# Shunpoco/mini-kube-scheduler

Measured on AMD Instinct MI355X. Metric: pod×node filter+score evals/sec and pods scheduled/sec at 100k nodes, 1/2/4/8 GPU, higher is better.
Workload: dtype u32; 1 GPU; C: 100000 nodes x 100000 pods (100000 per GPU, strong scaling), NU+NN, batched, every pair evaluated, node-sharded over 1 GPU; nodes=100000, pods=100000, pods_per_gpu=100000, plugins=NU+NN, parallelism=node-shard1

## Files before the change

mini-kube-scheduler_amd/csrc/ms_sweep_pp.hip:

```cpp
#include <hip/hip_ext.h>

#include <algorithm>
#include <cstdlib>

#include "ms_device.h"

namespace msgpu {

namespace {

template <typename F>
constexpr uint32_t truth3(F f) {
    uint32_t t = 0;
    for (int i = 0; i < 8; ++i)
        if (f((i >> 2) & 1, (i >> 1) & 1, i & 1)) t |= 1u << i;
    return t;
}
constexpr uint32_t kXnorAnd = truth3([](int a, int b, int c) { return c && a == b; });
constexpr uint32_t kSelect = truth3([](int a, int b, int c) { return c ? a : b; });

constexpr uint32_t kTailShare = 4;

constexpr int kPpWords = 4;
constexpr int kPpWordsSmall = 8;
constexpr int kPpMaxWaves = 16;
constexpr uint32_t kPpSmallGroups = 64u * kPpWordsSmall;

struct Word {
    uint32_t d0, d1, d2, d3;
    uint32_t sched, pres;
    uint32_t dsched, dpres;
    uint32_t hb;
};

struct Pod {
    uint32_t A;
    uint32_t s0, s1, s2, s3;
    uint32_t tol;
    uint32_t p0, p1, p2;
    uint32_t A0, A1, A2;
};

#define MS_BITOP3(a, b, c, imm) __builtin_amdgcn_bitop3_b32((a), (b), (c), (imm))

__device__ __forceinline__ uint32_t feasible(const Word &w, const Pod &q) {
    return MS_BITOP3(w.pres, w.sched, q.tol, kSelect);
}

__device__ __forceinline__ uint32_t match10(const Word &w, const Pod &q) {
    uint32_t m = MS_BITOP3(w.d0, q.s0, feasible(w, q), kXnorAnd);
    m = MS_BITOP3(w.d1, q.s1, m, kXnorAnd);
    m = MS_BITOP3(w.d2, q.s2, m, kXnorAnd);
    return MS_BITOP3(w.d3, q.s3, m, kXnorAnd);
}

__device__ __forceinline__ uint32_t last_lz(uint32_t m) {
    uint32_t s;
    asm("v_ffbh_u32 %0, %1" : "=v"(s) : "v"(m));
// ... 214 lines not shown
    uint32_t off, ns, nt;
};

__device__ __forceinline__ DigitLists digit_lists(const uint32_t *hdr, uint32_t d) {
    DigitLists L;
    L.off = hdr[d];
    L.nt = (hdr[d + 1] - L.off) / kCandTile;
    L.ns = hdr[kCandDigits + 1u + d];
    return L;
}

__device__ __forceinline__ uint32_t list_tiles(const DigitLists &L, bool tolerates) {
    return tolerates ? L.nt : L.ns;
}

struct ClassLanes {
    uint32_t beg, end;
    DigitLists L;
    u64 planes;
};

__device__ __forceinline__ ClassLanes class_lanes(const uint32_t *hdr, const uint32_t *rb, uint32_t base10,
                                                  uint32_t lane) {
    const uint32_t c = min(lane, kPpClasses);
    ClassLanes C;
    C.beg = rb[c];
    C.end = rb[c + 1];
    C.L = digit_lists(hdr, ((c >> 1) + base10) % kCandDigits);
    C.planes = __ballot(lane <= kPpClasses && C.beg < C.end &&
                        (c == kPpClasses || list_tiles(C.L, (c & 1u) != 0u) == 0u));
    return C;
}

__device__ __forceinline__ uint32_t lane_value(uint32_t v, uint32_t l) {
    return (uint32_t)__builtin_amdgcn_readlane((int)v, (int)l);
}

template <int NT>
__device__ __forceinline__ void sweep_list_pods(const uint32_t (&B)[3 * kPpWords], const uint2 *pinfo, uint32_t beg,
                                                uint32_t end, uint32_t lane, u64 *lds) {
    for (uint32_t pb = beg; pb < end; pb += 64) {
        const uint32_t nblk = min(64u, end - pb);
        const uint32_t a_l = lane < nblk ? pinfo[pb + lane].x : 0u;
        for (uint32_t j = 0; j < nblk; j += 8) {
            uint32_t r[8];
            if (nblk - j >= 8u) {
#pragma unroll
                for (int t = 0; t < 8; ++t) {
                    const uint32_t A = (uint32_t)__builtin_amdgcn_readlane((int)a_l, (int)(j + t));
                    uint32_t h = 0;
#pragma unroll
                    for (int i = 0; i < 3 * NT; ++i) h = max(h, mix32(B[i] + A));
                    r[t] = h;
                }
            } else {
#pragma unroll
                for (int t = 0; t < 8; ++t) {
                    r[t] = 0;
                    if (j + (uint32_t)t < nblk) {
                        const uint32_t A = (uint32_t)__builtin_amdgcn_readlane((int)a_l, (int)(j + t));
#pragma unroll
                        for (int i = 0; i < 3 * NT; ++i) r[t] = max(r[t], mix32(B[i] + A));
                    }
                }
            }
            const uint32_t u = reduce8(r, lane);
            const uint32_t pi = j + rev3(lane >> 3);
            if ((lane & 7u) == 0u && pi < nblk) atomicMax(&lds[pb + pi], (11ull << 32) | u);
        }
    }
}

__device__ __forceinline__ void sweep_list_tiles(uint32_t n, const uint32_t (&B)[3 * kPpWords], const uint2 *pinfo,
                                                 uint32_t beg, uint32_t end, uint32_t lane, u64 *lds) {
    switch (n) {
        case 1: sweep_list_pods<1>(B, pinfo, beg, end, lane, lds); break;
        case 2: sweep_list_pods<2>(B, pinfo, beg, end, lane, lds); break;
        case 3: sweep_list_pods<3>(B, pinfo, beg, end, lane, lds); break;
        default: sweep_list_pods<4>(B, pinfo, beg, end, lane, lds); break;
    }
}

__device__ __forceinline__ void load_list_tiles(const uint32_t *__restrict__ cand, uint32_t off, uint32_t t0,
                                                uint32_t nt, uint32_t waves, uint32_t lane,
                                                uint32_t (&B)[3 * kPpWords]) {
#pragma unroll
    for (int k = 0; k < kPpWords; ++k) {
        const uint32_t tile = t0 + ((uint32_t)k < nt ? (uint32_t)k * waves : 0u);
        const uint32_t *e = cand + kCandHeader + off + tile * kCandTile + lane;
#pragma unroll
        for (int i = 0; i < 3; ++i) B[3 * k + i] = e[i * 64];
    }
}

__device__ __forceinline__ void sweep_lists(const uint32_t *__restrict__ cand, const ClassLanes &C,
                                            const uint2 *pinfo, uint32_t wv, uint32_t waves, uint32_t lane,
                                            u64 *lds) {
    for (uint32_t s = 0; s < kPpClasses; s += 2) {
        const uint32_t b0 = lane_value(C.beg, s), b1 = lane_value(C.end, s), b2 = lane_value(C.end, s + 1u);
        if (b0 >= b2) continue;
        const DigitLists L = {lane_value(C.L.off, s), lane_value(C.L.ns, s), lane_value(C.L.nt, s)};
        const uint32_t ntile = list_tiles(L, b1 < b2);
        for (uint32_t t0 = wv; t0 < ntile; t0 += kPpWords * waves) {
            const uint32_t nt = min((uint32_t)kPpWords, (ntile - t0 + waves - 1u) / waves);
            const uint32_t ns = t0 < L.ns ? min((uint32_t)kPpWords, (L.ns - t0 + waves - 1u) / waves) : 0u;
            uint32_t B[3 * kPpWords];
            load_list_tiles(cand, L.off, t0, nt, waves, lane, B);
            if (ns != 0u && b0 < b1) sweep_list_tiles(ns, B, pinfo, b0, b1, lane, lds);
            if (b1 < b2) sweep_list_tiles(nt, B, pinfo, b1, b2, lane, lds);
        }
    }
}

template <int KW, int NW, int MODE, bool TAIL>
__device__ __forceinline__ void sweep_range(const Word (&W)[KW], const Word &Wt, uint32_t tpt, uint32_t tshare,
                                            uint32_t tidx, const uint2 *pinfo, const uint32_t *rb, bool runs,
                                            bool lists, const uint32_t *hdr, uint32_t base10, uint32_t np,
                                            uint32_t lane, u64 *lds) {
    constexpr bool RUN = MODE != kModeGen && NW > 0 && KW == kPpWords;
    const bool cut = lists || (RUN && runs);
    u64 todo = cut ? (2ull << kPpClasses) - 1ull : 1ull << kPpClasses;
    uint32_t cbeg = 0, cend = 0;
    if (lists) {
        const ClassLanes C = class_lanes(hdr, rb, base10, lane);
        cbeg = C.beg, cend = C.end, todo = C.planes;
    }
    for (; todo; todo &= todo - 1ull) {
        const uint32_t c = (uint32_t)__builtin_ctzll(todo);
        const uint32_t beg = lists ? lane_value(cbeg, c)
                             : cut ? (uint32_t)__builtin_amdgcn_readfirstlane((int)rb[c]) : 0u;
        const uint32_t end = lists ? lane_value(cend, c)
                             : cut ? (uint32_t)__builtin_amdgcn_readfirstlane((int)rb[c + 1]) : np;
        if (beg >= end) continue;
        uint32_t B[RUN ? NW * 3 : 1] = {};
        bool form = false;
        if constexpr (RUN)
            if (!lists && c < kPpClasses)
                form = run_setup<KW, NW>(W, (uint32_t)__builtin_amdgcn_readfirstlane((int)pinfo[beg].y), B);
        sweep_pods<KW, NW, MODE, TAIL>(W, Wt, tpt, tshare, tidx, pinfo, beg, end, form, B, lane, lds);
    }
}

__host__ __device__ inline uint32_t tail_pods(uint32_t ng, uint32_t waves) {
    if (ng == 0) return 0u;
    const uint32_t wlast = (ng + 63u) / 64u - 1u, tail_n = ng - wlast * 64u;
    const uint32_t tpt = tail_n <= 8u ? 8u : 0u;
    if (!tpt) return 0u;
    if (waves <= 4u) return tpt;
    const uint32_t wv_t = wlast % waves;
    const uint32_t tshare = kTailShare < waves - wv_t ? kTailShare : waves - wv_t;
    uint32_t L[4] = {0, 0, 0, 0};
    for (uint32_t w = 0; w < waves && w <= wlast; ++w) L[w & 3u] += 16u * ((wlast - w) / waves + 1u);
    auto mx = [&] {
        const uint32_t a = L[0] > L[1] ? L[0] : L[1], b = L[2] > L[3] ? L[2] : L[3];
        return a > b ? a : b;
    };
    const uint32_t m0 = mx();
    L[wv_t & 3u] -= 16u;
    const uint32_t eps = ((tpt == 8u ? 4u : tpt == 4u ? 8u : 12u) + tshare - 1u) / tshare;
    for (uint32_t i = 0; i < tshare; ++i) L[(wv_t + i) & 3u] += eps;
    return mx() < m0 ? tpt : 0u;
}

struct PpJob2 {
    const ms_pod_rec *pods;
    u64 *keys;
    uint32_t n_pods, nblk1;
};

template <int KW, bool TP>
__global__ __launch_bounds__(64 * kPpMaxWaves) void k_sweep_nunn_pp(
    const uint32_t *__restrict__ planes, uint32_t gstride, uint32_t n_groups, uint32_t node_base,
    const ms_pod_rec *__restrict__ pods1, uint32_t n_pods1, uint32_t chunk, uint32_t seed32, u64 *__restrict__ keys1,
    int atomic_keys, ms_result *__restrict__ results, uint32_t present, NodeTable tab, int commit,
    uint32_t pstride, ms_result_compact *__restrict__ resc, PpJob2 j2, int fix_ok, uint32_t xtra,
    const uint32_t *__restrict__ cand) {
    extern __shared__ u64 lds[];
    uint2 *pinfo = reinterpret_cast<uint2 *>(lds + chunk + (xtra ? 8u : 0u));
    const uint32_t lane = lane_id();
    const uint32_t wv = (uint32_t)__builtin_amdgcn_readfirstlane((int)(threadIdx.x >> 6));
    const bool second = j2.pods && blockIdx.x >= j2.nblk1;
    const ms_pod_rec *__restrict__ pods = second ? j2.pods : pods1;
    const uint32_t n_pods = second ? j2.n_pods : n_pods1;
    u64 *__restrict__ keys = second ? j2.keys : keys1;
    const uint32_t bi = second ? blockIdx.x - j2.nblk1 : blockIdx.x;
    const uint32_t pbeg = bi * chunk + min(bi, xtra) * 8u;
    const uint32_t pend = min(n_pods, pbeg + chunk + (bi < xtra ? 8u : 0u));
    const uint32_t np = pend > pbeg ? pend - pbeg : 0u;
    uint32_t *cnt = reinterpret_cast<uint32_t *>(pinfo + chunk + (xtra ? 8u : 0u));
    uint32_t *rb = cnt + 24, *sb = cnt + 48, *hdr = cnt + 72;
    const bool runs = KW == kPpWords && chunk >= kPpSortMin;
    const bool lists = runs && cand != nullptr && gridDim.y == 1u;
    if (!runs) {
        for (uint32_t i = threadIdx.x; i < np; i += blockDim.x) {
            lds[i] = 0;
            uint2 e = pod_entry(pods, pbeg + i, seed32, pstride, node_base % 10u);
            e.y |= i << 21;
            pinfo[i] = e;
        }
    } else {
        if (threadIdx.x < 24u) cnt[threadIdx.x] = 0u;
        if (lists)
            for (uint32_t i = threadIdx.x; i <= kCandClasses; i += blockDim.x) hdr[i] = cand[i];
        __syncthreads();
        for (uint32_t i = threadIdx.x; i < np; i += blockDim.x) {
            uint2 e = pod_entry(pods, pbeg + i, seed32, pstride, node_base % 10u);
            e.y |= atomicAdd(&cnt[pod_class(e.y)], 1u) << 21;
            reinterpret_cast<uint2 *>(lds)[i] = e;
        }
        __syncthreads();
        if (threadIdx.x <= kPpClasses) {
            uint32_t a = 0, b = 0, na = 0, nb = 0;
            for (uint32_t c = 0; c < kPpClasses; ++c) {
                const uint32_t n = cnt[c], full = lists ? n : n & ~7u;
                if (c == threadIdx.x) a = na, b = nb;
                na += full;
                nb += n - full;
            }
            if (threadIdx.x == kPpClasses) {
                a = na, b = nb;
                rb[kPpClasses + 1] = np;
            }
            rb[threadIdx.x] = a;
            sb[threadIdx.x] = na + b;
        }
        __syncthreads();
        for (uint32_t i = threadIdx.x; i < np; i += blockDim.x) {
            const uint2 e = reinterpret_cast<const uint2 *>(lds)[i];
            const uint32_t c = pod_class(e.y), rank = e.y >> 21;
            const uint32_t full = c < kPpClasses ? rb[c + 1] - rb[c] : 0u;
            const uint32_t pos = rank < full ? rb[c] + rank : sb[c] + (rank - full);
            pinfo[pos] = make_uint2(e.x, (e.y & 0x1FFFFFu) | (i << 21));
            lds[i] = 0;
        }
    }

    const uint32_t waves = blockDim.x >> 6;
    const uint32_t g0 = blockIdx.y * waves * 64u * KW;
    const uint32_t ng = min(n_groups - g0, waves * 64u * KW);
    const uint32_t wlast = (ng + 63u) / 64u - 1u, tail_n = ng - wlast * 64u;
    uint32_t tpt = TP ? tail_pods(ng, waves) : 0u;
    const uint32_t wv_t = wlast % waves, tshare = min(kTailShare, waves - wv_t);
    const bool owner = wv == wv_t;
    if (wv < wv_t || wv >= wv_t + tshare) tpt = 0u;
    Word W[KW], Wt;
    int nw = 0;
    bool over = false, misaligned = false;
#pragma unroll
    for (int k = 0; k < KW; ++k) {
        const uint32_t wi = k * waves + wv;
        const uint32_t gw = g0 + wi * 64u;
        const uint32_t g = gw + lane;
        const bool in = g < n_groups && !(tpt && owner && wi == wlast);
        if (gw < n_groups && !(tpt && owner && wi == wlast)) nw = k + 1;
        W[k].d0 = in ? planes[kPlaneD0 * gstride + g] : 0u;
        W[k].d1 = in ? planes[kPlaneD1 * gstride + g] : 0u;
        W[k].d2 = in ? planes[kPlaneD2 * gstride + g] : 0u;
        W[k].d3 = in ? planes[kPlaneD3 * gstride + g] : 0u;
        W[k].sched = in ? planes[kPlaneSched * gstride + g] : 0u;
        W[k].pres = in ? planes[kPlanePresent * gstride + g] : 0u;
        W[k].dsched = in ? planes[kPlaneDigitSched * gstride + g] : 0u;
        W[k].dpres = in ? planes[kPlaneDigitPres * gstride + g] : 0u;
        W[k].hb = (node_base + g * kGroupRows) * kG24;
        const uint32_t ov = in ? planes[kPlaneOver * gstride + g] : 0u;
        over = over || (ov & 1u) != 0u;
        misaligned = misaligned || (ov & 2u) != 0u;
    }
    {
        const uint32_t gi = tpt ? lane & ((64u / tpt) - 1u) : 0u;
        const uint32_t g = g0 + wlast * 64u + gi;
        const bool in = tpt && gi < tail_n;
        Wt.d0 = in ? planes[kPlaneD0 * gstride + g] : 0u;
        Wt.d1 = in ? planes[kPlaneD1 * gstride + g] : 0u;
        Wt.d2 = in ? planes[kPlaneD2 * gstride + g] : 0u;
        Wt.d3 = in ? planes[kPlaneD3 * gstride + g] : 0u;
        Wt.sched = in ? planes[kPlaneSched * gstride + g] : 0u;
        Wt.pres = in ? planes[kPlanePresent * gstride + g] : 0u;
        Wt.hb = (node_base + g * kGroupRows) * kG24;
        Wt.dsched = Wt.dpres = 0u;
        over = over || (in && (planes[kPlaneOver * gstride + g] & 1u) != 0u);
    }
    const bool gen = __ballot(over) != 0;
    const int mode = gen ? kModeGen : (fix_ok && __ballot(misaligned) == 0) ? kModeFix : kModeFast;
    __syncthreads();
    if (np && (nw || tpt)) {
        switch (nw * 6 + mode * 2 + (tpt ? 1 : 0)) {
#define MS_PP_CASE1(N, M, T)                                                                                     \
    case 6 * N + 2 * M + T:                                                                                      \
        if constexpr (N <= KW && (N > 0 || T))                                                                   \
            sweep_range<KW, (N <= KW ? N : KW), M, T>(W, Wt, tpt, tshare, wv - wv_t, pinfo, rb, runs, lists, hdr,   \
                                                      node_base % 10u, np, lane, lds);                          \
        break;
#define MS_PP_CASE(N)        \
    MS_PP_CASE1(N, 0, false) \
    MS_PP_CASE1(N, 0, true)  \
    MS_PP_CASE1(N, 1, false) \
    MS_PP_CASE1(N, 1, true)  \
    MS_PP_CASE1(N, 2, false) \
    MS_PP_CASE1(N, 2, true)
            MS_PP_CASE(0)
            MS_PP_CASE(1)
            MS_PP_CASE(2)
            MS_PP_CASE(3)
            MS_PP_CASE(4)
            MS_PP_CASE(5)
            MS_PP_CASE(6)
            MS_PP_CASE(7)
            MS_PP_CASE(8)
#undef MS_PP_CASE
#undef MS_PP_CASE1
            default:
                break;
        }
    }
    if constexpr (KW == kPpWords)
        if (np && lists)
            sweep_lists(cand, class_lanes(hdr, rb, node_base % 10u, lane), pinfo, wv, waves, lane, lds);
    __syncthreads();
    for (uint32_t i = threadIdx.x; i < np; i += blockDim.x) {
        const u64 v = lds[i];
        const uint2 pe = pinfo[i];
        const uint32_t po = pbeg + (pe.y >> 21);
        u64 key = present ? kKeyListed : 0ull;
        if (v) {
            const uint32_t h = (uint32_t)v;
            key = make_key((uint32_t)(v >> 32) - 1u, h, tb_unhash(pe.x, h));
        }
        if (keys) {
            if (!atomic_keys) keys[po] = key;
            else if (key) atomicMax(&keys[po], key);
        }
        if (results || resc) {
            const ms_result r = decode_key(key, (int8_t)(pe.y >> 8), nullptr, 0, present);
            if (results) {
                results[po] = r;
            } else {
                ms_result_compact rc;
                rc.node = r.node;
                rc.score = (uint16_t)r.score;
                rc.code = (uint8_t)r.code;
                rc.plugin_mask = (uint8_t)r.plugin_mask;
                resc[po] = rc;
            }
            if (commit && r.code == MS_CODE_SUCCESS) {
                if (resc) {
                    const ms_pod_rec z = {};
                    add_pod(tab, (uint32_t)r.node - tab.base, z, +1);
                } else {
                    add_pod(tab, (uint32_t)r.node - tab.base, pods[po], +1);
                }
            }
        }
    }
}

__host__ __device__ inline uint32_t cdiv(uint32_t a, uint32_t b) { return (a + b - 1) / b; }

__device__ __forceinline__ void build_group(const NodeTable &t, uint32_t g) {
    uint32_t d[4] = {0, 0, 0, 0}, sched = 0, pres = 0, isdig = 0, misal = 0;
    for (uint32_t s = 0; s < kGroupRows; ++s) {
        const uint32_t r = g * kGroupRows + s;
        if (r >= t.cap) break;
        const uint32_t f = t.flags[r], dg = t.digit[r];
        const uint32_t v = dg <= 9u ? dg : 15u;
#pragma unroll
        for (int b = 0; b < 4; ++b) d[b] |= ((v >> b) & 1u) << s;
        if (!(f & kNodeAbsent)) {
            pres |= 1u << s;
            if (!(f & kNodeUnschedulable)) sched |= 1u << s;
            if (v <= 9u) {
                isdig |= 1u << s;
                if (v != (t.base + r) % 10u) misal = 2u;
            }
        }
    }
    uint32_t over = misal;
#pragma unroll
    for (int v = 0; v < 10; ++v) {
        const uint32_t m = pres & ((v & 1) ? d[0] : ~d[0]) & ((v & 2) ? d[1] : ~d[1]) & ((v & 4) ? d[2] : ~d[2]) &
                           ((v & 8) ? d[3] : ~d[3]);
        over |= __popc(m) > 3 ? 1u : 0u;
    }
    const uint32_t st = t.gcap;
    t.planes[kPlaneDigitPres * st + g] = pres & isdig;
    t.planes[kPlaneDigitSched * st + g] = sched & isdig;
    t.planes[kPlaneOver * st + g] = over;
// ... 73 lines not shown
            total += wsum[w];
        }
        uint32_t pos = done + before + incl - k;
        while (m) {
            const uint32_t slot = (uint32_t)__builtin_ctz(m);
            m &= m - 1u;
            const uint32_t e = (t.base + g * kGroupRows + slot) * kG24;
            if (pos == 0u) first = e;
            if (pos < len) ent[pos] = e;
            ++pos;
        }
        done += total;
        __syncthreads();
    }
    for (uint32_t i = len + tid; i < padded; i += kCandThreads) ent[i] = first;
}

}

hipError_t launch_build_planes(const NodeTable &t, uint32_t *cand, const NodeDelta *d_deltas, uint32_t n,
                               hipStream_t s) {
    if (!t.planes) return hipSuccess;
    if (!d_deltas) n = t.gcap;
    if (n == 0) return hipSuccess;
    hipLaunchKernelGGL(k_build_planes, dim3(cdiv(n, 256)), dim3(256), 0, s, t, d_deltas, n);
    hipError_t e = hipGetLastError();
    if (e != hipSuccess || !cand) return e;
    hipLaunchKernelGGL(k_build_cand, dim3(kCandClasses), dim3(kCandThreads), 0, s, t, cand);
    return hipGetLastError();
}

constexpr uint32_t kPpMaxChunk = 2048;

namespace {
hipError_t sweep_pp_impl(const NodeTable &t, const uint32_t *cand, uint32_t n_rows, const ms_pod_rec *pods, uint32_t n_pods,
                         uint32_t seed32, unsigned long long *keys, ms_result *results, uint32_t present, int num_cus,
                         hipStream_t s, int commit, hipEvent_t done, uint32_t pstride, ms_result_compact *resc,
                         const ms_pod_rec *pods2 = nullptr, uint32_t n_pods2 = 0, unsigned long long *keys2 = nullptr) {
    if (n_pods == 0 && n_pods2 == 0) return done ? hipEventRecord(done, s) : hipSuccess;
    const uint32_t n_all = n_pods + (pods2 ? n_pods2 : 0u);
    if (!t.planes) return hipErrorInvalidValue;
    const uint32_t n_groups = cdiv(n_rows, kGroupRows);
    const char *wenv = getenv("MINISCHED_PP_WORDS");
    const uint32_t cus_ = (uint32_t)(num_cus > 0 ? num_cus : 256);
    bool small = n_groups <= kPpSmallGroups && n_all >= 1024u * cus_ && !getenv("MINISCHED_PP_WAVES");
    if (wenv) small = n_groups <= kPpSmallGroups && atoi(wenv) == 8;
    const uint32_t KW = small ? (uint32_t)kPpWordsSmall : (uint32_t)kPpWords;
    const uint32_t waves_needed = std::max(1u, cdiv(n_groups, 64u * KW));
    uint32_t W = 1;
    if (waves_needed == 2) W = 2;
    else if (waves_needed > 1)
        while (W < std::max(4u, waves_needed) && W < (uint32_t)kPpMaxWaves) W *= 2;
    if (const char *w = getenv("MINISCHED_PP_WAVES")) W = (uint32_t)std::min(16, std::max(1, atoi(w)));
    if (!keys) W = std::max(W, std::min<uint32_t>(kPpMaxWaves, waves_needed));
    const uint32_t gy = std::max(1u, cdiv(n_groups, W * 64u * KW));
    const uint32_t cus = (uint32_t)(num_cus > 0 ? num_cus : 256);
    auto chunk_for = [&](uint32_t per_cu) {
        const uint32_t resident = std::max(1u, per_cu * cus / gy);
        return cdiv(cdiv(n_all, resident), 8) * 8;
    };
    uint32_t chunk = chunk_for(std::max(1u, 32u / W));
    if (32u / W > 1u && chunk_for(std::max(1u, 16u / W)) <= 1024u) chunk = chunk_for(std::max(1u, 16u / W));
    chunk = std::min(std::max(chunk, 8u), kPpMaxChunk);
    uint32_t nblk1 = cdiv(n_pods, chunk), xtra = 0;
    if ((!pods2 || n_pods2 == n_pods) && gy == 1 && W <= 4u) {
        const uint32_t slots = (16u / W) * cus / (pods2 ? 2u : 1u);
        const uint32_t cb = (n_pods / slots) / 8u * 8u;
        if (cb >= 8u && cb + 8u <= kPpMaxChunk && n_pods > cb * slots) {
            const uint32_t nx = cdiv(n_pods - cb * slots, 8u);
            if (nx <= slots) {
                chunk = cb;
                xtra = nx;
                nblk1 = slots;
            }
        }
    }
    const dim3 grid(nblk1 + (pods2 ? (xtra ? nblk1 : cdiv(n_pods2, chunk)) : 0u), gy);
    constexpr int fix_ok = 1;
    const PpJob2 j2 = {pods2, reinterpret_cast<u64 *>(keys2), n_pods2, nblk1};
    if (pods2 && (gy > 1 || results || resc || !keys || !keys2)) return hipErrorInvalidValue;
    if (gy > 1) {
        if (!keys || resc) return hipErrorInvalidValue;
        hipError_t e = hipMemsetAsync(keys, 0, sizeof(unsigned long long) * n_pods, s);
        if (e != hipSuccess) return e;
        hipLaunchKernelGGL((k_sweep_nunn_pp<kPpWords, false>), grid, dim3(64 * W),
                           chunk * (sizeof(u64) + sizeof(uint2)) + kPpSortWords * sizeof(uint32_t), s, t.planes,
                           t.gcap, n_groups, t.base, pods, n_pods, chunk, seed32, keys, 1, (ms_result *)nullptr, present,
                           t, 0, (uint32_t)sizeof(ms_pod_rec), (ms_result_compact *)nullptr, PpJob2{}, fix_ok, 0u,
                           (const uint32_t *)nullptr);
        e = hipGetLastError();
        if (e == hipSuccess && results) e = launch_decode(pods, n_pods, keys, nullptr, present, results, s);
        if (e == hipSuccess && results && commit) e = launch_apply_binds(t, pods, n_pods, results, s);
        if (e == hipSuccess && done) e = hipEventRecord(done, s);
        return e;
    }
    const uint32_t lds = (chunk + (xtra ? 8u : 0u)) * (sizeof(u64) + sizeof(uint2)) + kPpSortWords * sizeof(uint32_t);
    unsigned long long *kk = (results || resc) ? nullptr : keys;
    const int cm = (results || resc) ? commit : 0;
    const bool tp = KW == (uint32_t)kPpWords && tail_pods(n_groups, W) != 0u;
#define MS_PP_LAUNCH(KWV, TPV)                                                                                     \
    hipExtLaunchKernelGGL((k_sweep_nunn_pp<KWV, TPV>), grid, dim3(64 * W), lds, s, nullptr, done, 0, t.planes, t.gcap, \
                          n_groups, t.base, pods, n_pods, chunk, seed32, kk, 0, results, present, t, cm, pstride, resc, j2, \
                          fix_ok, xtra, cand)
    if (KW == (uint32_t)kPpWordsSmall) {
        MS_PP_LAUNCH(kPpWordsSmall, false);
    } else {
        if (tp) MS_PP_LAUNCH(kPpWords, true);
        else MS_PP_LAUNCH(kPpWords, false);
    }
#undef MS_PP_LAUNCH
    return hipGetLastError();
}
}

hipError_t launch_sweep_pp(const NodeTable &t, const uint32_t *cand, uint32_t n_rows, const ms_pod_rec *pods, uint32_t n_pods,
                           uint32_t seed32, unsigned long long *keys, ms_result *results, uint32_t present,
                           int num_cus, hipStream_t s, int commit, hipEvent_t done) {
    return sweep_pp_impl(t, cand, n_rows, pods, n_pods, seed32, keys, results, present, num_cus, s, commit, done,
                         (uint32_t)sizeof(ms_pod_rec), nullptr);
}

hipError_t launch_sweep_pp2(const NodeTable &t, const uint32_t *cand, uint32_t n_rows, const ms_pod_rec *pods1, uint32_t n1,
                            unsigned long long *keys1, const ms_pod_rec *pods2, uint32_t n2, unsigned long long *keys2,
                            uint32_t seed32, uint32_t present, int num_cus, hipStream_t s, hipEvent_t done) {
    if (n_rows > kPpMaxFusedRows) return hipErrorInvalidValue;
    return sweep_pp_impl(t, cand, n_rows, pods1, n1, seed32, keys1, nullptr, present, num_cus, s, 0, done,
                         (uint32_t)sizeof(ms_pod_rec), nullptr, pods2, n2, keys2);
}

hipError_t launch_sweep_pp_compact(const NodeTable &t, const uint32_t *cand, uint32_t n_rows, const ms_pod_compact *pods, uint32_t n_pods,
                                   uint32_t seed32, ms_result_compact *results, uint32_t present, int num_cus,
                                   hipStream_t s) {
    static_assert(sizeof(ms_pod_compact) == 8 && sizeof(ms_result_compact) == 8, "compact records");
    if (n_rows > kPpMaxFusedRows || !results) return hipErrorInvalidValue;
    return sweep_pp_impl(t, cand, n_rows, reinterpret_cast<const ms_pod_rec *>(pods), n_pods, seed32, nullptr, nullptr,
                         present, num_cus, s, 1, nullptr, (uint32_t)sizeof(ms_pod_compact), results);
}

}
```

Before: 57270 billion pod×node evals/s.

## Deal list tiles and pod ranges across wave groups in sweep_lists

Waves are now split into up to four groups. Each group takes a share of the pod blocks per digit, rotated between digits so the load stays balanced, and each wave holds up to G×4 candidate tiles in registers instead of 4. The intent is more register reuse of the loaded tiles across pods and fewer redundant tile loads per pod. The cost is higher register pressure from larger B arrays, which may hurt occupancy, plus a runtime-looped tail path. The change also adds optional timeline instrumentation that is compiled out by default.

After: 59650 billion pod×node evals/s, median of 6. +4.1%, better.

```diff
diff --git a/mini-kube-scheduler_amd/csrc/ms_pp_deal.h b/mini-kube-scheduler_amd/csrc/ms_pp_deal.h
--- /dev/null
+++ b/mini-kube-scheduler_amd/csrc/ms_pp_deal.h
@@ -0,0 +1,105 @@
+#pragma once
+
+#include <cstdint>
+
+#if !defined(__HIPCC__) && !defined(__host__)
+#define __host__
+#define __device__
+#define MS_PP_DEAL_OWN_ATTRS
+#endif
+
+namespace msgpu {
+
+constexpr uint32_t kDealTiles = 4;
+
+struct WaveDeal {
+    uint32_t groups;
+    uint32_t gshift;
+    uint32_t group;
+    uint32_t index;
+    uint32_t wpg;
+    uint32_t inv;
+};
+
+__host__ __device__ inline uint32_t deal_groups(uint32_t waves, uint32_t want) {
+    if (waves % 4u) return 1u;
+    uint32_t g = want >= 4u ? 4u : want >= 2u ? 2u : 1u;
+    while (g > 1u && (waves / 4u) % g) g >>= 1;
+    return g;
+}
+
+__host__ __device__ inline WaveDeal wave_deal(uint32_t wv, uint32_t waves, uint32_t want) {
+    WaveDeal D;
+    D.groups = deal_groups(waves, want);
+    D.gshift = D.groups >> 1;
+    D.group = (wv >> 2) & (D.groups - 1u);
+    D.index = (wv & 3u) + 4u * ((wv >> 2) >> D.gshift);
+    D.wpg = waves >> D.gshift;
+    D.inv = 0xFFFFFFFFu / D.wpg + 1u;
+    return D;
+}
+
+__host__ __device__ inline uint32_t deal_div(const WaveDeal &D, uint32_t n) {
+    return D.wpg == 1u ? n : (uint32_t)(((unsigned long long)n * D.inv) >> 32);
+}
+
+__host__ __device__ inline uint32_t deal_hold(const WaveDeal &D) { return kDealTiles << D.gshift; }
+__host__ __device__ inline uint32_t deal_pass_tiles(const WaveDeal &D) { return deal_hold(D) * D.wpg; }
+
+struct DigitDeal {
+    uint32_t off, nt, ns;
+};
+
+__host__ __device__ inline DigitDeal deal_digit(const WaveDeal &D, uint32_t ntile, uint32_t ns_all) {
+    DigitDeal X;
+    X.off = D.index;
+    const uint32_t qt = deal_div(D, ntile), rt = ntile - qt * D.wpg;
+    const uint32_t qs = deal_div(D, ns_all), rs = ns_all - qs * D.wpg;
+    X.nt = qt + (X.off < rt ? 1u : 0u);
+    X.ns = qs + (X.off < rs ? 1u : 0u);
+    return X;
+}
+
+struct TileDeal {
+    uint32_t first, nt, ns;
+};
+
+__host__ __device__ inline TileDeal deal_tiles(const WaveDeal &D, const DigitDeal &X, uint32_t pass) {
+    const uint32_t hold = deal_hold(D), done = pass * hold;
+    TileDeal T;
+    T.first = done * D.wpg + X.off;
+    T.nt = X.nt > done ? X.nt - done : 0u;
+    if (T.nt > hold) T.nt = hold;
+    T.ns = X.ns > done ? X.ns - done : 0u;
+    if (T.ns > T.nt) T.ns = T.nt;
+    return T;
+}
+
+struct PodDeal {
+    uint32_t beg, end;
+};
+
+__host__ __device__ inline PodDeal deal_pods(const WaveDeal &D, uint32_t prot, uint32_t beg, uint32_t end) {
+    const uint32_t nb = end > beg ? (end - beg + 7u) >> 3 : 0u;
+    const uint32_t base = nb >> D.gshift, extra = nb & (D.groups - 1u);
+    const uint32_t gi = (D.group - prot) & (D.groups - 1u);
+    const uint32_t start = gi * base + (gi < extra ? gi : extra), cnt = base + (gi < extra ? 1u : 0u);
+    PodDeal P;
+    P.beg = beg + 8u * start;
+    P.end = beg + 8u * (start + cnt);
+    if (P.end > end) P.end = end;
+    if (cnt == 0u || P.beg > P.end) P.beg = P.end;
+    return P;
+}
+
+__host__ __device__ inline uint32_t deal_prot_next(const WaveDeal &D, uint32_t prot, uint32_t n) {
+    return (prot + ((n + 7u) >> 3)) & (D.groups - 1u);
+}
+
+}
+
+#ifdef MS_PP_DEAL_OWN_ATTRS
+#undef __host__
+#undef __device__
+#undef MS_PP_DEAL_OWN_ATTRS
+#endif
diff --git a/mini-kube-scheduler_amd/csrc/ms_sweep_pp.hip b/mini-kube-scheduler_amd/csrc/ms_sweep_pp.hip
--- a/mini-kube-scheduler_amd/csrc/ms_sweep_pp.hip
+++ b/mini-kube-scheduler_amd/csrc/ms_sweep_pp.hip
@@ -4,10 +4,36 @@
 #include <cstdlib>
 
 #include "ms_device.h"
+#include "ms_pp_deal.h"
+
+#ifdef MS_PP_TIMELINE
+#include <cstdio>
+#include <vector>
+#endif
 
 namespace msgpu {
 
 namespace {
+
+#ifdef MS_PP_TIMELINE
+constexpr uint32_t kTlEntry = 0, kTlSorted = 1, kTlPlanes = 2, kTlBarrier = 3, kTlPlaneSweep = 4;
+constexpr uint32_t kTlDigit = 5;
+constexpr uint32_t kTlDone = 35, kTlFinalBarrier = 36, kTlExit = 37, kTlHwId = 38, kTlSlots = 40;
+__device__ unsigned long long *g_pp_tl;
+__device__ __forceinline__ void pp_stamp(uint32_t slot, bool hwid = false) {
+    unsigned long long *tl = g_pp_tl;
+    if (!tl) return;
+    const uint32_t waves = blockDim.x >> 6, wg = blockIdx.x * gridDim.y + blockIdx.y;
+    const unsigned long long t =
+        hwid ? (unsigned long long)__builtin_amdgcn_s_getreg((31 << 11) | 4) : __builtin_amdgcn_s_memrealtime();
+    if ((threadIdx.x & 63u) == 0u) tl[((size_t)wg * waves + (threadIdx.x >> 6)) * kTlSlots + slot] = t;
+}
+#define MS_PP_STAMP(slot) pp_stamp(slot)
+#define MS_PP_TILES_USED(B) asm volatile("" ::"v"((B)[0]), "v"((B)[sizeof(B) / sizeof((B)[0]) - 1]))
+#else
+#define MS_PP_STAMP(slot) ((void)0)
+#define MS_PP_TILES_USED(B) ((void)0)
+#endif
 
 template <typename F>
 constexpr uint32_t truth3(F f) {
@@ -22,8 +48,10 @@
 constexpr uint32_t kTailShare = 4;
 
 constexpr int kPpWords = 4;
+static_assert(kDealTiles == (uint32_t)kPpWords, "a group's tiles take the registers of a wave's words");
 constexpr int kPpWordsSmall = 8;
 constexpr int kPpMaxWaves = 16;
+constexpr uint32_t kPpGroups = 4;
 constexpr uint32_t kPpSmallGroups = 64u * kPpWordsSmall;
 
 struct Word {
@@ -308,8 +336,8 @@
     return (uint32_t)__builtin_amdgcn_readlane((int)v, (int)l);
 }
 
-template <int NT>
-__device__ __forceinline__ void sweep_list_pods(const uint32_t (&B)[3 * kPpWords], const uint2 *pinfo, uint32_t beg,
+template <int NMAX, int NT>
+__device__ __forceinline__ void sweep_list_pods(const uint32_t (&B)[3 * NMAX], const uint2 *pinfo, uint32_t beg,
                                                 uint32_t end, uint32_t lane, u64 *lds) {
     for (uint32_t pb = beg; pb < end; pb += 64) {
         const uint32_t nblk = min(64u, end - pb);
@@ -325,7 +353,7 @@
                     for (int i = 0; i < 3 * NT; ++i) h = max(h, mix32(B[i] + A));
                     r[t] = h;
                 }
-            } else {
+            } else if constexpr (NT <= kPpWords) {
 #pragma unroll
                 for (int t = 0; t < 8; ++t) {
                     r[t] = 0;
@@ -334,6 +362,18 @@
 #pragma unroll
                         for (int i = 0; i < 3 * NT; ++i) r[t] = max(r[t], mix32(B[i] + A));
                     }
+                }
+            } else {
+#pragma unroll
+                for (int t = 0; t < 8; ++t) r[t] = 0;
+#pragma unroll 1
+                for (uint32_t t = 0; t < nblk - j; ++t) {
+                    const uint32_t A = (uint32_t)__builtin_amdgcn_readlane((int)a_l, (int)(j + t));
+                    uint32_t h = 0;
+#pragma unroll
+                    for (int i = 0; i < 3 * NT; ++i) h = max(h, mix32(B[i] + A));
+#pragma unroll
+                    for (int u = 0; u < 8; ++u) r[u] = t == (uint32_t)u ? h : r[u];
                 }
             }
             const uint32_t u = reduce8(r, lane);
@@ -343,43 +383,59 @@
     }
 }
 
-__device__ __forceinline__ void sweep_list_tiles(uint32_t n, const uint32_t (&B)[3 * kPpWords], const uint2 *pinfo,
+template <int NMAX, int N = 1>
+__device__ __forceinline__ void sweep_list_tiles(uint32_t n, const uint32_t (&B)[3 * NMAX], const uint2 *pinfo,
                                                  uint32_t beg, uint32_t end, uint32_t lane, u64 *lds) {
-    switch (n) {
-        case 1: sweep_list_pods<1>(B, pinfo, beg, end, lane, lds); break;
-        case 2: sweep_list_pods<2>(B, pinfo, beg, end, lane, lds); break;
-        case 3: sweep_list_pods<3>(B, pinfo, beg, end, lane, lds); break;
-        default: sweep_list_pods<4>(B, pinfo, beg, end, lane, lds); break;
-    }
-}
-
+    if constexpr (N >= NMAX) {
+        sweep_list_pods<NMAX, NMAX>(B, pinfo, beg, end, lane, lds);
+    } else {
+        if (n == (uint32_t)N) sweep_list_pods<NMAX, N>(B, pinfo, beg, end, lane, lds);
+        else sweep_list_tiles<NMAX, N + 1>(n, B, pinfo, beg, end, lane, lds);
+    }
+}
+
+template <int NMAX>
 __device__ __forceinline__ void load_list_tiles(const uint32_t *__restrict__ cand, uint32_t off, uint32_t t0,
-                                                uint32_t nt, uint32_t waves, uint32_t lane,
-                                                uint32_t (&B)[3 * kPpWords]) {
-#pragma unroll
-    for (int k = 0; k < kPpWords; ++k) {
-        const uint32_t tile = t0 + ((uint32_t)k < nt ? (uint32_t)k * waves : 0u);
+                                                uint32_t nt, uint32_t stride, uint32_t lane,
+                                                uint32_t (&B)[3 * NMAX]) {
+#pragma unroll
+    for (int k = 0; k < NMAX; ++k) {
+        const uint32_t tile = t0 + ((uint32_t)k < nt ? (uint32_t)k * stride : 0u);
         const uint32_t *e = cand + kCandHeader + off + tile * kCandTile + lane;
 #pragma unroll
         for (int i = 0; i < 3; ++i) B[3 * k + i] = e[i * 64];
     }
 }
 
+template <int G>
 __device__ __forceinline__ void sweep_lists(const uint32_t *__restrict__ cand, const ClassLanes &C,
                                             const uint2 *pinfo, uint32_t wv, uint32_t waves, uint32_t lane,
                                             u64 *lds) {
+    constexpr int NMAX = G * kPpWords;
+    const WaveDeal D = wave_deal(wv, waves, (uint32_t)G);
+    uint32_t prot = 0;
     for (uint32_t s = 0; s < kPpClasses; s += 2) {
         const uint32_t b0 = lane_value(C.beg, s), b1 = lane_value(C.end, s), b2 = lane_value(C.end, s + 1u);
         if (b0 >= b2) continue;
         const DigitLists L = {lane_value(C.L.off, s), lane_value(C.L.ns, s), lane_value(C.L.nt, s)};
         const uint32_t ntile = list_tiles(L, b1 < b2);
-        for (uint32_t t0 = wv; t0 < ntile; t0 += kPpWords * waves) {
-            const uint32_t nt = min((uint32_t)kPpWords, (ntile - t0 + waves - 1u) / waves);
-            const uint32_t ns = t0 < L.ns ? min((uint32_t)kPpWords, (L.ns - t0 + waves - 1u) / waves) : 0u;
-            uint32_t B[3 * kPpWords];
-            load_list_tiles(cand, L.off, t0, nt, waves, lane, B);
-            if (ns != 0u && b0 < b1) sweep_list_tiles(ns, B, pinfo, b0, b1, lane, lds);
-            if (b1 < b2) sweep_list_tiles(nt, B, pinfo, b1, b2, lane, lds);
+        const PodDeal P0 = deal_pods(D, prot, b0, b1);
+        prot = deal_prot_next(D, prot, b1 - b0);
+        const PodDeal P1 = deal_pods(D, prot, b1, b2);
+        prot = deal_prot_next(D, prot, b2 - b1);
+        const DigitDeal X = deal_digit(D, ntile, L.ns);
+        if (P0.beg >= P0.end && P1.beg >= P1.end) continue;
+        for (uint32_t pass = 0;; ++pass) {
+            const TileDeal T = deal_tiles(D, X, pass);
+            if (T.nt == 0u) break;
+            uint32_t B[3 * NMAX];
+            MS_PP_STAMP(kTlDigit + 3u * (s >> 1));
+            load_list_tiles<NMAX>(cand, L.off, T.first, T.nt, D.wpg, lane, B);
+            MS_PP_TILES_USED(B);
+            MS_PP_STAMP(kTlDigit + 3u * (s >> 1) + 1u);
+            if (T.ns != 0u && P0.beg < P0.end) sweep_list_tiles<NMAX>(T.ns, B, pinfo, P0.beg, P0.end, lane, lds);
+            if (P1.beg < P1.end) sweep_list_tiles<NMAX>(T.nt, B, pinfo, P1.beg, P1.end, lane, lds);
+            MS_PP_STAMP(kTlDigit + 3u * (s >> 1) + 2u);
         }
     }
 }
@@ -440,7 +496,7 @@
     uint32_t n_pods, nblk1;
 };
 
-template <int KW, bool TP>
+template <int KW, bool TP, int G>
 __global__ __launch_bounds__(64 * kPpMaxWaves) void k_sweep_nunn_pp(
     const uint32_t *__restrict__ planes, uint32_t gstride, uint32_t n_groups, uint32_t node_base,
     const ms_pod_rec *__restrict__ pods1, uint32_t n_pods1, uint32_t chunk, uint32_t seed32, u64 *__restrict__ keys1,
@@ -448,6 +504,7 @@
     uint32_t pstride, ms_result_compact *__restrict__ resc, PpJob2 j2, int fix_ok, uint32_t xtra,
     const uint32_t *__restrict__ cand) {
     extern __shared__ u64 lds[];
+    MS_PP_STAMP(kTlEntry);
     uint2 *pinfo = reinterpret_cast<uint2 *>(lds + chunk + (xtra ? 8u : 0u));
     const uint32_t lane = lane_id();
     const uint32_t wv = (uint32_t)__builtin_amdgcn_readfirstlane((int)(threadIdx.x >> 6));
@@ -507,6 +564,7 @@
         }
     }
 
+    MS_PP_STAMP(kTlSorted);
     const uint32_t waves = blockDim.x >> 6;
     const uint32_t g0 = blockIdx.y * waves * 64u * KW;
     const uint32_t ng = min(n_groups - g0, waves * 64u * KW);
@@ -554,7 +612,9 @@
     }
     const bool gen = __ballot(over) != 0;
     const int mode = gen ? kModeGen : (fix_ok && __ballot(misaligned) == 0) ? kModeFix : kModeFast;
+    MS_PP_STAMP(kTlPlanes);
     __syncthreads();
+    MS_PP_STAMP(kTlBarrier);
     if (np && (nw || tpt)) {
         switch (nw * 6 + mode * 2 + (tpt ? 1 : 0)) {
 #define MS_PP_CASE1(N, M, T)                                                                                     \
@@ -585,10 +645,13 @@
                 break;
         }
     }
+    MS_PP_STAMP(kTlPlaneSweep);
     if constexpr (KW == kPpWords)
         if (np && lists)
-            sweep_lists(cand, class_lanes(hdr, rb, node_base % 10u, lane), pinfo, wv, waves, lane, lds);
+            sweep_lists<G>(cand, class_lanes(hdr, rb, node_base % 10u, lane), pinfo, wv, waves, lane, lds);
+    MS_PP_STAMP(kTlDone);
     __syncthreads();
+    MS_PP_STAMP(kTlFinalBarrier);
     for (uint32_t i = threadIdx.x; i < np; i += blockDim.x) {
         const u64 v = lds[i];
         const uint2 pe = pinfo[i];
@@ -624,6 +687,10 @@
             }
         }
     }
+    MS_PP_STAMP(kTlExit);
+#ifdef MS_PP_TIMELINE
+    pp_stamp(kTlHwId, true);
+#endif
 }
 
 __host__ __device__ inline uint32_t cdiv(uint32_t a, uint32_t b) { return (a + b - 1) / b; }
@@ -810,11 +877,25 @@
     constexpr int fix_ok = 1;
     const PpJob2 j2 = {pods2, reinterpret_cast<u64 *>(keys2), n_pods2, nblk1};
     if (pods2 && (gy > 1 || results || resc || !keys || !keys2)) return hipErrorInvalidValue;
+#ifdef MS_PP_TIMELINE
+    static unsigned long long *d_tl = nullptr;
+    static size_t tl_cap = 0;
+    const char *tlf = getenv("MS_PP_TIMELINE");
+    const size_t tl_n = (size_t)grid.x * grid.y * W * kTlSlots;
+    if (tlf && tl_n > tl_cap) {
+        (void)hipFree(d_tl);
+        if (hipMalloc(&d_tl, tl_n * sizeof(*d_tl)) != hipSuccess) return hipErrorOutOfMemory;
+        tl_cap = tl_n;
+    }
+    if (tlf && hipMemsetAsync(d_tl, 0, tl_n * sizeof(*d_tl), s) != hipSuccess) return hipErrorUnknown;
+    unsigned long long *tl_arg = tlf ? d_tl : nullptr;
+    if (hipMemcpyToSymbol(HIP_SYMBOL(g_pp_tl), &tl_arg, sizeof(tl_arg)) != hipSuccess) return hipErrorUnknown;
+#endif
     if (gy > 1) {
         if (!keys || resc) return hipErrorInvalidValue;
         hipError_t e = hipMemsetAsync(keys, 0, sizeof(unsigned long long) * n_pods, s);
         if (e != hipSuccess) return e;
-        hipLaunchKernelGGL((k_sweep_nunn_pp<kPpWords, false>), grid, dim3(64 * W),
+        hipLaunchKernelGGL((k_sweep_nunn_pp<kPpWords, false, 1>), grid, dim3(64 * W),
                            chunk * (sizeof(u64) + sizeof(uint2)) + kPpSortWords * sizeof(uint32_t), s, t.planes,
                            t.gcap, n_groups, t.base, pods, n_pods, chunk, seed32, keys, 1, (ms_result *)nullptr, present,
                            t, 0, (uint32_t)sizeof(ms_pod_rec), (ms_result_compact *)nullptr, PpJob2{}, fix_ok, 0u,
@@ -829,17 +910,37 @@
     unsigned long long *kk = (results || resc) ? nullptr : keys;
     const int cm = (results || resc) ? commit : 0;
     const bool tp = KW == (uint32_t)kPpWords && tail_pods(n_groups, W) != 0u;
-#define MS_PP_LAUNCH(KWV, TPV)                                                                                     \
-    hipExtLaunchKernelGGL((k_sweep_nunn_pp<KWV, TPV>), grid, dim3(64 * W), lds, s, nullptr, done, 0, t.planes, t.gcap, \
+    const uint32_t gsel = deal_groups(W, kPpGroups);
+#define MS_PP_LAUNCH(KWV, TPV, GV)                                                                                     \
+    hipExtLaunchKernelGGL((k_sweep_nunn_pp<KWV, TPV, GV>), grid, dim3(64 * W), lds, s, nullptr, done, 0, t.planes, t.gcap, \
                           n_groups, t.base, pods, n_pods, chunk, seed32, kk, 0, results, present, t, cm, pstride, resc, j2, \
                           fix_ok, xtra, cand)
     if (KW == (uint32_t)kPpWordsSmall) {
-        MS_PP_LAUNCH(kPpWordsSmall, false);
+        MS_PP_LAUNCH(kPpWordsSmall, false, 1);
+    } else if (gsel == 4) {
+        if (tp) MS_PP_LAUNCH(kPpWords, true, 4);
+        else MS_PP_LAUNCH(kPpWords, false, 4);
+    } else if (gsel == 2) {
+        if (tp) MS_PP_LAUNCH(kPpWords, true, 2);
+        else MS_PP_LAUNCH(kPpWords, false, 2);
     } else {
-        if (tp) MS_PP_LAUNCH(kPpWords, true);
-        else MS_PP_LAUNCH(kPpWords, false);
+        if (tp) MS_PP_LAUNCH(kPpWords, true, 1);
+        else MS_PP_LAUNCH(kPpWords, false, 1);
     }
 #undef MS_PP_LAUNCH
+#ifdef MS_PP_TIMELINE
+    if (tlf) {
+        std::vector<unsigned long long> h(tl_n);
+        if (hipStreamSynchronize(s) != hipSuccess || hipMemcpy(h.data(), d_tl, tl_n * sizeof(*d_tl), hipMemcpyDeviceToHost) != hipSuccess)
+            return hipErrorUnknown;
+        if (FILE *f = fopen(tlf, "wb")) {
+            const uint32_t hd[4] = {grid.x * grid.y, W, kTlSlots, 0u};
+            fwrite(hd, sizeof(hd), 1, f);
+            fwrite(h.data(), sizeof(h[0]), tl_n, f);
+            fclose(f);
+        }
+    }
+#endif
     return hipGetLastError();
 }
 }
```

## Accumulate list-sweep scores in per-lane LDS table instead of cross-lane reduce

Applied to the files above, without the earlier changes.

Adds an optional per-lane LDS table (64 words per pod) in which each lane accumulates its max score with workgroup-scoped LDS atomics. This replaces the per-8-pod cross-lane reduce8 and the 64-bit atomicMax in the candidate-list sweep. A post-pass reduces each row with a vector load plus DPP row shuffles and merges the result into the per-pod key, only for classes the lists covered. It raises the dynamic LDS size via hipFuncSetAttribute and is gated on an occupancy fit check. The cost is much more LDS per workgroup, a zeroing pass and extra synchronisation.

Measured after the change: 57670 billion pod×node evals/s before, 60310 billion pod×node evals/s after (median of 6 runs). 1.05x the previous value.

```diff
diff --git a/mini-kube-scheduler_amd/csrc/ms_sweep_pp.hip b/mini-kube-scheduler_amd/csrc/ms_sweep_pp.hip
--- a/mini-kube-scheduler_amd/csrc/ms_sweep_pp.hip
+++ b/mini-kube-scheduler_amd/csrc/ms_sweep_pp.hip
@@ -1,6 +1,7 @@
 #include <hip/hip_ext.h>
 
 #include <algorithm>
+#include <atomic>
 #include <cstdlib>
 
 #include "ms_device.h"
@@ -304,13 +305,29 @@
     return C;
 }
 
+__device__ __forceinline__ bool list_covered(const uint32_t *hdr, uint32_t c, uint32_t base10) {
+    return c < kPpClasses && list_tiles(digit_lists(hdr, ((c >> 1) + base10) % kCandDigits), (c & 1u) != 0u) != 0u;
+}
+
 __device__ __forceinline__ uint32_t lane_value(uint32_t v, uint32_t l) {
     return (uint32_t)__builtin_amdgcn_readlane((int)v, (int)l);
 }
 
-template <int NT>
+__device__ __forceinline__ void lds_max_u32(uint32_t *p, uint32_t v) {
+    __hip_atomic_fetch_max(p, v, __ATOMIC_RELAXED, __HIP_MEMORY_SCOPE_WORKGROUP);
+}
+
+template <int LT>
+__device__ __forceinline__ void table_put(uint32_t *row, const uint32_t (&r)[8], uint32_t n) {
+    static_assert(LT == 64, "a word to a lane");
+#pragma unroll
+    for (int t = 0; t < 8; ++t)
+        if ((uint32_t)t < n) lds_max_u32(row + t * LT, r[t]);
+}
+
+template <int NT, int LT>
 __device__ __forceinline__ void sweep_list_pods(const uint32_t (&B)[3 * kPpWords], const uint2 *pinfo, uint32_t beg,
-                                                uint32_t end, uint32_t lane, u64 *lds) {
+                                                uint32_t end, uint32_t lane, u64 *lds, uint32_t *tabl) {
     for (uint32_t pb = beg; pb < end; pb += 64) {
         const uint32_t nblk = min(64u, end - pb);
         const uint32_t a_l = lane < nblk ? pinfo[pb + lane].x : 0u;
@@ -325,6 +342,7 @@
                     for (int i = 0; i < 3 * NT; ++i) h = max(h, mix32(B[i] + A));
                     r[t] = h;
                 }
+                if constexpr (LT != 0) table_put<LT>(tabl + (pb + j) * LT, r, 8u);
             } else {
 #pragma unroll
                 for (int t = 0; t < 8; ++t) {
@@ -335,22 +353,37 @@
                         for (int i = 0; i < 3 * NT; ++i) r[t] = max(r[t], mix32(B[i] + A));
                     }
                 }
-            }
-            const uint32_t u = reduce8(r, lane);
-            const uint32_t pi = j + rev3(lane >> 3);
-            if ((lane & 7u) == 0u && pi < nblk) atomicMax(&lds[pb + pi], (11ull << 32) | u);
-        }
-    }
-}
-
+                if constexpr (LT != 0) table_put<LT>(tabl + (pb + j) * LT, r, nblk - j);
+            }
+            if constexpr (LT == 0) {
+                const uint32_t u = reduce8(r, lane);
+                const uint32_t pi = j + rev3(lane >> 3);
+                if ((lane & 7u) == 0u && pi < nblk) atomicMax(&lds[pb + pi], (11ull << 32) | u);
+            }
+        }
+    }
+}
+
+template <int LT>
 __device__ __forceinline__ void sweep_list_tiles(uint32_t n, const uint32_t (&B)[3 * kPpWords], const uint2 *pinfo,
-                                                 uint32_t beg, uint32_t end, uint32_t lane, u64 *lds) {
+                                                 uint32_t beg, uint32_t end, uint32_t lane, u64 *lds, uint32_t *tabl) {
     switch (n) {
-        case 1: sweep_list_pods<1>(B, pinfo, beg, end, lane, lds); break;
-        case 2: sweep_list_pods<2>(B, pinfo, beg, end, lane, lds); break;
-        case 3: sweep_list_pods<3>(B, pinfo, beg, end, lane, lds); break;
-        default: sweep_list_pods<4>(B, pinfo, beg, end, lane, lds); break;
-    }
+        case 1: sweep_list_pods<1, LT>(B, pinfo, beg, end, lane, lds, tabl); break;
+        case 2: sweep_list_pods<2, LT>(B, pinfo, beg, end, lane, lds, tabl); break;
+        case 3: sweep_list_pods<3, LT>(B, pinfo, beg, end, lane, lds, tabl); break;
+        default: sweep_list_pods<4, LT>(B, pinfo, beg, end, lane, lds, tabl); break;
+    }
+}
+
+template <int LT>
+__device__ __forceinline__ uint32_t table_rowmax(const uint32_t *tab, uint32_t i, uint32_t sub) {
+    const uint4 q = *reinterpret_cast<const uint4 *>(tab + i * LT + sub * 4u);
+    uint32_t m = max(max(q.x, q.y), max(q.z, q.w));
+    m = max(m, (uint32_t)__builtin_amdgcn_update_dpp(0, (int)m, 0x111, 0xF, 0xF, false));
+    m = max(m, (uint32_t)__builtin_amdgcn_update_dpp(0, (int)m, 0x112, 0xF, 0xF, false));
+    m = max(m, (uint32_t)__builtin_amdgcn_update_dpp(0, (int)m, 0x114, 0xF, 0xF, false));
+    m = max(m, (uint32_t)__builtin_amdgcn_update_dpp(0, (int)m, 0x118, 0xF, 0xF, false));
+    return m;
 }
 
 __device__ __forceinline__ void load_list_tiles(const uint32_t *__restrict__ cand, uint32_t off, uint32_t t0,
@@ -365,9 +398,10 @@
     }
 }
 
+template <int LT>
 __device__ __forceinline__ void sweep_lists(const uint32_t *__restrict__ cand, const ClassLanes &C,
                                             const uint2 *pinfo, uint32_t wv, uint32_t waves, uint32_t lane,
-                                            u64 *lds) {
+                                            u64 *lds, uint32_t *tabl) {
     for (uint32_t s = 0; s < kPpClasses; s += 2) {
         const uint32_t b0 = lane_value(C.beg, s), b1 = lane_value(C.end, s), b2 = lane_value(C.end, s + 1u);
         if (b0 >= b2) continue;
@@ -378,8 +412,8 @@
             const uint32_t ns = t0 < L.ns ? min((uint32_t)kPpWords, (L.ns - t0 + waves - 1u) / waves) : 0u;
             uint32_t B[3 * kPpWords];
             load_list_tiles(cand, L.off, t0, nt, waves, lane, B);
-            if (ns != 0u && b0 < b1) sweep_list_tiles(ns, B, pinfo, b0, b1, lane, lds);
-            if (b1 < b2) sweep_list_tiles(nt, B, pinfo, b1, b2, lane, lds);
+            if (ns != 0u && b0 < b1) sweep_list_tiles<LT>(ns, B, pinfo, b0, b1, lane, lds, tabl);
+            if (b1 < b2) sweep_list_tiles<LT>(nt, B, pinfo, b1, b2, lane, lds, tabl);
         }
     }
 }
@@ -440,14 +474,14 @@
     uint32_t n_pods, nblk1;
 };
 
-template <int KW, bool TP>
+template <int KW, bool TP, int LT>
 __global__ __launch_bounds__(64 * kPpMaxWaves) void k_sweep_nunn_pp(
     const uint32_t *__restrict__ planes, uint32_t gstride, uint32_t n_groups, uint32_t node_base,
     const ms_pod_rec *__restrict__ pods1, uint32_t n_pods1, uint32_t chunk, uint32_t seed32, u64 *__restrict__ keys1,
     int atomic_keys, ms_result *__restrict__ results, uint32_t present, NodeTable tab, int commit,
     uint32_t pstride, ms_result_compact *__restrict__ resc, PpJob2 j2, int fix_ok, uint32_t xtra,
     const uint32_t *__restrict__ cand) {
-    extern __shared__ u64 lds[];
+    extern __shared__ __attribute__((aligned(16))) u64 lds[];
     uint2 *pinfo = reinterpret_cast<uint2 *>(lds + chunk + (xtra ? 8u : 0u));
     const uint32_t lane = lane_id();
     const uint32_t wv = (uint32_t)__builtin_amdgcn_readfirstlane((int)(threadIdx.x >> 6));
@@ -463,6 +497,11 @@
     uint32_t *rb = cnt + 24, *sb = cnt + 48, *hdr = cnt + 72;
     const bool runs = KW == kPpWords && chunk >= kPpSortMin;
     const bool lists = runs && cand != nullptr && gridDim.y == 1u;
+    uint32_t *ltab = hdr + 24;
+    if constexpr (LT != 0) {
+        uint4 *z = reinterpret_cast<uint4 *>(ltab);
+        for (uint32_t i = threadIdx.x; i < np * (LT / 4); i += blockDim.x) z[i] = make_uint4(0u, 0u, 0u, 0u);
+    }
     if (!runs) {
         for (uint32_t i = threadIdx.x; i < np; i += blockDim.x) {
             lds[i] = 0;
@@ -587,8 +626,24 @@
     }
     if constexpr (KW == kPpWords)
         if (np && lists)
-            sweep_lists(cand, class_lanes(hdr, rb, node_base % 10u, lane), pinfo, wv, waves, lane, lds);
+            sweep_lists<LT>(cand, class_lanes(hdr, rb, node_base % 10u, lane), pinfo, wv, waves, lane, lds,
+                            ltab + lane);
     __syncthreads();
+    if constexpr (LT != 0) {
+        if (np && lists) {
+            constexpr uint32_t G = LT / 4;
+            const uint32_t sub = threadIdx.x % G;
+            for (uint32_t i0 = 0; i0 < np; i0 += blockDim.x / G) {
+                const uint32_t i = i0 + threadIdx.x / G;
+                const uint32_t m = table_rowmax<LT>(ltab, min(i, np - 1u), sub);
+                if (sub == G - 1u && i < np) {
+                    if (list_covered(hdr, pod_class(pinfo[i].y), node_base % 10u))
+                        lds[i] = umax64(lds[i], (11ull << 32) | m);
+                }
+            }
+        }
+        __syncthreads();
+    }
     for (uint32_t i = threadIdx.x; i < np; i += blockDim.x) {
         const u64 v = lds[i];
         const uint2 pe = pinfo[i];
@@ -763,7 +818,35 @@
 
 constexpr uint32_t kPpMaxChunk = 2048;
 
+constexpr uint32_t kPpLdsPerCu = 160u * 1024u;
+constexpr int kPpLaneWords = 64;
+
+__host__ inline uint32_t pp_lds_bytes(uint32_t cap, uint32_t lt) {
+    return cap * (uint32_t)(sizeof(u64) + sizeof(uint2)) + kPpSortWords * (uint32_t)sizeof(uint32_t) +
+           cap * lt * (uint32_t)sizeof(uint32_t);
+}
+
+__host__ inline bool lane_table_fits(uint32_t chunk, uint32_t xtra, uint32_t W, uint32_t per_cu) {
+    if (chunk < kPpSortMin || W > (uint32_t)kPpMaxWaves) return false;
+    const uint32_t wg = (pp_lds_bytes(chunk + (xtra ? 8u : 0u), (uint32_t)kPpLaneWords) + 2047u) / 2048u * 2048u;
+    return wg * per_cu <= kPpLdsPerCu;
+}
+
 namespace {
+template <auto kernel>
+hipError_t allow_lds() {
+    static std::atomic<bool> set[64];
+    int dev = 0;
+    hipError_t e = hipGetDevice(&dev);
+    if (e != hipSuccess) return e;
+    if (dev < 0 || dev >= 64 || !set[dev].load(std::memory_order_acquire)) {
+        e = hipFuncSetAttribute(reinterpret_cast<const void *>(kernel), hipFuncAttributeMaxDynamicSharedMemorySize,
+                                (int)kPpLdsPerCu);
+        if (e == hipSuccess && dev >= 0 && dev < 64) set[dev].store(true, std::memory_order_release);
+    }
+    return e;
+}
+
 hipError_t sweep_pp_impl(const NodeTable &t, const uint32_t *cand, uint32_t n_rows, const ms_pod_rec *pods, uint32_t n_pods,
                          uint32_t seed32, unsigned long long *keys, ms_result *results, uint32_t present, int num_cus,
                          hipStream_t s, int commit, hipEvent_t done, uint32_t pstride, ms_result_compact *resc,
@@ -790,8 +873,12 @@
         const uint32_t resident = std::max(1u, per_cu * cus / gy);
         return cdiv(cdiv(n_all, resident), 8) * 8;
     };
-    uint32_t chunk = chunk_for(std::max(1u, 32u / W));
-    if (32u / W > 1u && chunk_for(std::max(1u, 16u / W)) <= 1024u) chunk = chunk_for(std::max(1u, 16u / W));
+    uint32_t per_cu = std::max(1u, 32u / W);
+    uint32_t chunk = chunk_for(per_cu);
+    if (32u / W > 1u && chunk_for(std::max(1u, 16u / W)) <= 1024u) {
+        per_cu = std::max(1u, 16u / W);
+        chunk = chunk_for(per_cu);
+    }
     chunk = std::min(std::max(chunk, 8u), kPpMaxChunk);
     uint32_t nblk1 = cdiv(n_pods, chunk), xtra = 0;
     if ((!pods2 || n_pods2 == n_pods) && gy == 1 && W <= 4u) {
@@ -803,6 +890,7 @@
                 chunk = cb;
                 xtra = nx;
                 nblk1 = slots;
+                per_cu = 16u / W;
             }
         }
     }
@@ -814,7 +902,7 @@
         if (!keys || resc) return hipErrorInvalidValue;
         hipError_t e = hipMemsetAsync(keys, 0, sizeof(unsigned long long) * n_pods, s);
         if (e != hipSuccess) return e;
-        hipLaunchKernelGGL((k_sweep_nunn_pp<kPpWords, false>), grid, dim3(64 * W),
+        hipLaunchKernelGGL((k_sweep_nunn_pp<kPpWords, false, 0>), grid, dim3(64 * W),
                            chunk * (sizeof(u64) + sizeof(uint2)) + kPpSortWords * sizeof(uint32_t), s, t.planes,
                            t.gcap, n_groups, t.base, pods, n_pods, chunk, seed32, keys, 1, (ms_result *)nullptr, present,
                            t, 0, (uint32_t)sizeof(ms_pod_rec), (ms_result_compact *)nullptr, PpJob2{}, fix_ok, 0u,
@@ -825,19 +913,26 @@
         if (e == hipSuccess && done) e = hipEventRecord(done, s);
         return e;
     }
-    const uint32_t lds = (chunk + (xtra ? 8u : 0u)) * (sizeof(u64) + sizeof(uint2)) + kPpSortWords * sizeof(uint32_t);
+    const bool table = KW == (uint32_t)kPpWords && cand != nullptr && lane_table_fits(chunk, xtra, W, per_cu);
+    const uint32_t lds = pp_lds_bytes(chunk + (xtra ? 8u : 0u), table ? (uint32_t)kPpLaneWords : 0u);
     unsigned long long *kk = (results || resc) ? nullptr : keys;
     const int cm = (results || resc) ? commit : 0;
     const bool tp = KW == (uint32_t)kPpWords && tail_pods(n_groups, W) != 0u;
-#define MS_PP_LAUNCH(KWV, TPV)                                                                                     \
-    hipExtLaunchKernelGGL((k_sweep_nunn_pp<KWV, TPV>), grid, dim3(64 * W), lds, s, nullptr, done, 0, t.planes, t.gcap, \
-                          n_groups, t.base, pods, n_pods, chunk, seed32, kk, 0, results, present, t, cm, pstride, resc, j2, \
-                          fix_ok, xtra, cand)
+#define MS_PP_LAUNCH(KWV, TPV, LTV)                                                                                 \
+    hipExtLaunchKernelGGL((k_sweep_nunn_pp<KWV, TPV, LTV>), grid, dim3(64 * W), lds, s, nullptr, done, 0, t.planes,   \
+                          t.gcap, n_groups, t.base, pods, n_pods, chunk, seed32, kk, 0, results, present, t, cm, pstride, \
+                          resc, j2, fix_ok, xtra, cand)
     if (KW == (uint32_t)kPpWordsSmall) {
-        MS_PP_LAUNCH(kPpWordsSmall, false);
+        MS_PP_LAUNCH(kPpWordsSmall, false, 0);
+    } else if (table) {
+        const hipError_t e = tp ? allow_lds<k_sweep_nunn_pp<kPpWords, true, kPpLaneWords>>()
+                                : allow_lds<k_sweep_nunn_pp<kPpWords, false, kPpLaneWords>>();
+        if (e != hipSuccess) return e;
+        if (tp) MS_PP_LAUNCH(kPpWords, true, kPpLaneWords);
+        else MS_PP_LAUNCH(kPpWords, false, kPpLaneWords);
     } else {
-        if (tp) MS_PP_LAUNCH(kPpWords, true);
-        else MS_PP_LAUNCH(kPpWords, false);
+        if (tp) MS_PP_LAUNCH(kPpWords, true, 0);
+        else MS_PP_LAUNCH(kPpWords, false, 0);
     }
 #undef MS_PP_LAUNCH
     return hipGetLastError();
```
